# Lcrypto/mod-interleaveavx_multithreads-FAID

Hardware: AMD Instinct MI355X
Metric: decoded Gb/s @ 10 iters, 50G-PON LDPC; FER match vs AVX512 ref (higher is better)
Workload: dtype i8

## Files before the change

include/lnsfaid.h:

```cpp
#ifndef LNSFAID_H
#define LNSFAID_H

#include <stddef.h>
#include <stdint.h>

#ifdef __cplusplus
extern "C" {
#endif

#define LNSFAID_GROUP 32

#define LNSFAID_OK 0
#define LNSFAID_E_INVAL (-1)
#define LNSFAID_E_CODE (-2)
#define LNSFAID_E_NOMEM (-3)
#define LNSFAID_E_HIP (-4)
#define LNSFAID_E_NODEVICE (-5)
#define LNSFAID_E_INTERNAL (-6)

typedef struct lnsfaid_code {
    int32_t n_var;
    int32_t n_check;
    int32_t n_edges;
    int32_t z;
// ... 281 lines not shown
int lnsfaid_allreduce_counters(lnsfaid_ctx* ctx, uint64_t counters[4]);

int lnsfaid_select_kernel(lnsfaid_ctx* ctx, int32_t rows_per_lane);
int lnsfaid_kernel_rows_per_lane(const lnsfaid_ctx* ctx);

int lnsfaid_select_waves(lnsfaid_ctx* ctx, int32_t waves_per_codeword);
int lnsfaid_kernel_waves(const lnsfaid_ctx* ctx);

#define LNSFAID_MSG_REGISTERS 1
#define LNSFAID_MSG_HBM 2
int lnsfaid_select_message_store(lnsfaid_ctx* ctx, int32_t where);
int lnsfaid_message_store(const lnsfaid_ctx* ctx);

#define LNSFAID_ZERO_SHIFT_ON 1
#define LNSFAID_ZERO_SHIFT_OFF 2
#define LNSFAID_ZERO_SHIFT_LOOP 3
#define LNSFAID_ZERO_SHIFT_STATIC 4
#define LNSFAID_ZERO_SHIFT_WINDOWED 5
int lnsfaid_select_zero_shift(lnsfaid_ctx* ctx, int32_t mode);
int lnsfaid_zero_shift_groups(const lnsfaid_ctx* ctx, int32_t* groups, int32_t n);
int lnsfaid_window_free(const lnsfaid_ctx* ctx);
int lnsfaid_code_zero_shift_order(const lnsfaid_code* code, int32_t* groups, int32_t* order);

int lnsfaid_code_bf_walk(const lnsfaid_code* code, int32_t col_weight, uint32_t* full, uint32_t* flipped, uint32_t* fixed, int32_t* info);

int lnsfaid_kernel_residency(lnsfaid_ctx* ctx, int32_t* workgroups_per_cu, int32_t* lds_limit);


int lnsfaid_kernel_time(lnsfaid_ctx* ctx, double* out_ms, uint64_t* out_launches, int32_t reset);

void* lnsfaid_stream(lnsfaid_ctx* ctx);

const char* lnsfaid_strerror(int err);
const char* lnsfaid_last_hip_error(void);
const char* lnsfaid_version(void);

#ifdef __cplusplus
}
#endif
#endif
```

mod-interleaveavx_multithreads-faid_amd/csrc/lnsfaid_capi.hip:

```cpp
#include <hip/hip_runtime.h>

#include <dlfcn.h>
#include <rccl/rccl.h>

#include <cstdio>
#include <cstdlib>
#include <cstring>
#include <new>
#include <vector>

#include "lnsfaid_device.h"
#include "lnsfaid_line.h"
#include "lnsfaid_burst.h"
#include "lnsfaid_quantise.h"
#include "lnsfaid_swar.h"
#include "lnsfaid_launch.h"

#include <atomic>
#include <chrono>
#include <condition_variable>
#include <mutex>
#include <thread>
struct LfCombiner;
static thread_local char g_hip_err[256] = "";
// ... 45 lines not shown
    int32_t* d_status[2] = { nullptr, nullptr };
    uint32_t* d_remaining = nullptr;
    int32_t* d_live = nullptr;
    unsigned long long* d_counters = nullptr;
    uint32_t* h_remaining = nullptr;
    unsigned long long* h_counters = nullptr;
    int8_t* d_io_in = nullptr;
    int8_t* d_io_out = nullptr;
    lnsfaid_group_stats* d_io_stats = nullptr;
    lnsfaid_codeword_stats* d_io_cw_stats = nullptr;
    uint8_t* d_pk_in = nullptr;
    uint32_t* d_pk_out = nullptr;
    lnsfaid_group_stats* d_pk_stats = nullptr;
    uint32_t* d_ln_payload = nullptr;
    lnsfaid_line_stats* d_ln_stats = nullptr;
    LfBurstDesc* d_burst_desc = nullptr;
    LfBurstDesc* h_burst_desc = nullptr;
    uint32_t* d_burst_ones = nullptr;
    int early_stop = LNSFAID_STOP_GROUP;
    int rows_per_lane = 0;
    int waves_per_cw = 0;
    int msg_store = 0;
    int zero_shift = 0;
    mutable int static_code = -1;
    struct LfCombiner* comb = nullptr;
    int comb_slot = -1;
    const void* checked_fn[6] = {};
    int resident_wg[4] = {}, lds_wg[4] = {};
    void* comm = nullptr;
    bool comm_owned = false;
    unsigned long long* d_reduce = nullptr;
    double kernel_ms = 0.0;
    uint64_t kernel_launches = 0;
    uint32_t* d_fe_seeds = nullptr;
    unsigned long long* d_fe_draws = nullptr;
    int8_t* d_fe_codeword = nullptr;
    int8_t* d_fe_frames = nullptr;
    int8_t* d_fe_input = nullptr;
    size_t fe_frames_streams = 0;
    int fe_interleave = 1;
    int fe_exact = 0;
    int fe_prefec = 0;
    unsigned long long* d_fe_prefec_frames = nullptr;
    unsigned long long* d_fe_prefec_acc = nullptr;
    uint2* d_cap_cnt = nullptr;
    unsigned long long* d_cap_meta = nullptr;
// ... 321 lines not shown
    return LNSFAID_OK;
}

extern "C" int lnsfaid_create(lnsfaid_ctx** out, const lnsfaid_code* code, const lnsfaid_cfg* cfg, int32_t device,
                              size_t max_groups)
{
    if (!out || !code || !cfg || max_groups == 0 || max_groups > ((size_t)1 << 24)) return LNSFAID_E_INVAL;
    *out = nullptr;
    lnsfaid_ctx* ctx = new (std::nothrow) lnsfaid_ctx();
    if (!ctx) return LNSFAID_E_NOMEM;
    ctx->device = device;
    ctx->max_groups = max_groups;
    if (const char* e = getenv("LNSFAID_ROWS_PER_LANE"))
        ctx->rows_per_lane = (e[0] == '2') ? 2 : 0;
    if (const char* e = getenv("LNSFAID_WAVES_PER_CODEWORD"))
        ctx->waves_per_cw = (e[0] == '2') ? 2 : 0;
    if (const char* e = getenv("LNSFAID_FRONTEND_EXACT"))
        ctx->fe_exact = (e[0] == '1') ? 1 : 0;
    if (const char* e = getenv("LNSFAID_MSG_STORE"))
        ctx->msg_store = (e[0] == 'h') ? LNSFAID_MSG_HBM : ((e[0] == 'r') ? LNSFAID_MSG_REGISTERS : 0);
    if (const char* e = getenv("LNSFAID_ZERO_SHIFT"))
        ctx->zero_shift = (e[0] == 'o' && e[1] == 'f') ? LNSFAID_ZERO_SHIFT_OFF
                          : (e[0] == 'l' ? LNSFAID_ZERO_SHIFT_LOOP : (e[0] == 'w' ? LNSFAID_ZERO_SHIFT_WINDOWED : 0));
    g_live_contexts.fetch_add(1, std::memory_order_relaxed);
    const int rc = create_impl(ctx, code, cfg);
    if (rc) { lnsfaid_destroy(ctx); return rc; }
    ctx->comb_slot = comb_join(ctx);
    *out = ctx;
    return LNSFAID_OK;
}

extern "C" int lnsfaid_set_cfg(lnsfaid_ctx* ctx, const lnsfaid_cfg* cfg)
{
    if (!ctx || !cfg) return LNSFAID_E_INVAL;
    LfDevCfg n;
    int rc = build_cfg(cfg, &n);
    if (rc) return rc;
    rc = check_code_for_method(&ctx->hcode, n.method);
    if (rc) return rc;
    if (memcmp(&n, &ctx->hcfg, sizeof(n)) == 0) return LNSFAID_OK;
    HIP_TRY(hipSetDevice(ctx->device));
    HIP_TRY(hipStreamSynchronize(ctx->stream));
    if (n.W != ctx->hcfg.W) {
        build_wcols(&ctx->hcode, n.W);
        HIP_TRY(hipMemcpy(ctx->d_code, &ctx->hcode, sizeof(LfDevCode), hipMemcpyHostToDevice));
    }
// ... 66 lines not shown
static int layer_zero_groups(const lnsfaid_ctx* ctx, int br) { return (ctx->hcode.zinst[br] >> 8) & 0xff; }
static bool zero_shift_possible(const lnsfaid_ctx* ctx)
{
    if (!use_kernel4(ctx) || use_kernel5(ctx) || !use_msg_registers(ctx)) return false;
    if (ctx->hcfg.method < 1 || ctx->hcfg.method > 5) return false;
    for (int br = 0; br < ctx->hcode.nbr; ++br)
        if (layer_zero_groups(ctx, br) >= 1) return true;
    return false;
}
static bool use_zero_shift(const lnsfaid_ctx* ctx) { return ctx->zero_shift != LNSFAID_ZERO_SHIFT_OFF && zero_shift_possible(ctx); }

static bool static_layers_possible(const lnsfaid_ctx* ctx)
{
    if (ctx->static_code < 0) ctx->static_code = lf_decode4s_matches(&ctx->hcode);
    return ctx->static_code == 1 && zero_shift_possible(ctx);
}
static bool use_static_layers(const lnsfaid_ctx* ctx)
{
    return use_zero_shift(ctx) && ctx->zero_shift != LNSFAID_ZERO_SHIFT_LOOP && static_layers_possible(ctx);
}
static bool use_window_free(const lnsfaid_ctx* ctx)
{
    return use_static_layers(ctx) && ctx->zero_shift != LNSFAID_ZERO_SHIFT_WINDOWED && ctx->hcfg.floor_iter_thresh < 0;
}

extern "C" int lnsfaid_select_zero_shift(lnsfaid_ctx* ctx, int32_t mode)
{
    if (!ctx || mode < 0 || mode > LNSFAID_ZERO_SHIFT_WINDOWED) return LNSFAID_E_INVAL;
    if ((mode == LNSFAID_ZERO_SHIFT_ON || mode == LNSFAID_ZERO_SHIFT_LOOP) && !zero_shift_possible(ctx)) return LNSFAID_E_INVAL;
    if ((mode == LNSFAID_ZERO_SHIFT_STATIC || mode == LNSFAID_ZERO_SHIFT_WINDOWED) && !static_layers_possible(ctx)) return LNSFAID_E_INVAL;
    ctx->zero_shift = mode;
    return LNSFAID_OK;
}

extern "C" int lnsfaid_zero_shift_groups(const lnsfaid_ctx* ctx, int32_t* groups, int32_t n)
{
    if (!ctx || n < 0 || (n > 0 && !groups)) return LNSFAID_E_INVAL;
    const bool on = use_zero_shift(ctx);
    for (int br = 0; br < n; ++br) groups[br] = (on && br < ctx->hcode.nbr) ? layer_zero_groups(ctx, br) : 0;
    return on ? (use_static_layers(ctx) ? 2 : 1) : 0;
}

extern "C" int lnsfaid_window_free(const lnsfaid_ctx* ctx)
{
    if (!ctx) return LNSFAID_E_INVAL;
    return use_window_free(ctx) ? 1 : 0;
// ... 53 lines not shown
static bool cw_possible(const lnsfaid_ctx* ctx) { return ctx->waves_per_cw != 2 && use_kernel4(ctx); }

static bool packed_kernel(const lnsfaid_ctx* ctx) { return use_kernel4(ctx) && !use_kernel5(ctx); }

enum { LF_ENTRY_GROUP = LNSFAID_STOP_GROUP, LF_ENTRY_CW = LNSFAID_STOP_CODEWORD, LF_ENTRY_PACKED = 2 , LF_ENTRY_LINE = 4, LF_ENTRY_BURST };
static int decode_entry(int rule, bool packed) { return rule + (packed ? LF_ENTRY_PACKED : 0); }
struct LfInst {
    const void* fn;
    int threads;
};

static LfInst select_kernel(const lnsfaid_ctx* ctx, int entry)
{
    const int m = ctx->hcfg.method, ef = ctx->hcfg.ef, rm = use_msg_registers(ctx) ? 1 : 0;
    LfInst k = { nullptr, lf_decode4_threads() };
    switch (entry) {
    case LF_ENTRY_PACKED + LF_ENTRY_GROUP: k.fn = lf_decode4p_func(m, ef, rm, 0); break;
    case LF_ENTRY_PACKED + LF_ENTRY_CW: k.fn = lf_decode4p_func(m, ef, rm, 1); break;
    case LF_ENTRY_CW: if (cw_possible(ctx)) k.fn = lf_decode4cw_func(m, ef, rm); break;
    case LF_ENTRY_LINE: k.fn = lf_decode4l_func(m, ef, rm); break;
    case LF_ENTRY_BURST: k.fn = lf_decode4b_func(m, ef, rm); break;
    default:
        if (use_kernel5(ctx)) { k.fn = lf_decode5_func(m); k.threads = lf_decode5_threads(); }
        else if (use_window_free(ctx)) k.fn = lf_decode4w_func(m);
        else if (use_static_layers(ctx)) k.fn = lf_decode4s_func(m);
        else if (use_zero_shift(ctx)) k.fn = lf_decode4z_func(m);
        else if (use_kernel4(ctx)) k.fn = lf_decode4_func(m, ef, rm);
        else { k.fn = lf_decode_func(m, ctx->hcfg.uniform_w); k.threads = lf_decode_threads(); }
    }
    return k;
}

extern "C" int lnsfaid_select_message_store(lnsfaid_ctx* ctx, int32_t where)
{
    if (!ctx || where < 0 || where > LNSFAID_MSG_HBM) return LNSFAID_E_INVAL;
    if (where == LNSFAID_MSG_REGISTERS && !msg_registers_possible(ctx)) return LNSFAID_E_INVAL;
    ctx->msg_store = where;
    return LNSFAID_OK;
}

extern "C" int lnsfaid_message_store(const lnsfaid_ctx* ctx)
{
    if (!ctx) return LNSFAID_E_INVAL;
    if (!use_kernel4(ctx)) return LNSFAID_MSG_HBM;
    return use_msg_registers(ctx) ? LNSFAID_MSG_REGISTERS : LNSFAID_MSG_HBM;
}
// ... 431 lines not shown
            std::lock_guard<std::mutex> lk(cb->m);
            cb->slots[slot].state = LF_SLOT_FREE;
            cb->members -= 1;
            last = cb->members == 0;
            if (last) cb->stop = true;
            cb->cv_work.notify_all();
        }
        if (!last) return;
        if (g_comb[cb->device] == cb) g_comb[cb->device] = nullptr;
    }
    for (auto& th : cb->worker) if (th.joinable()) th.join();
    static const bool trace = getenv("LNSFAID_TRACE") != nullptr;
    if (trace && cb->batches)
        fprintf(stderr, "[lnsfaid] call combiner of device %d: %llu calls in %llu batches (%.1f per batch); per batch %.3f ms gathering, %.3f ms copies + decode\n",
                cb->device, (unsigned long long)cb->calls, (unsigned long long)cb->batches, (double)cb->calls / (double)cb->batches,
                cb->gather_ms / (double)cb->batches, cb->device_ms / (double)cb->batches);
    for (auto P : cb->pool) if (P) lnsfaid_destroy(P);
    if (cb->h_in) { (void)hipHostFree(cb->h_in); (void)hipHostFree(cb->h_out); (void)hipHostFree(cb->h_status); (void)hipHostFree(cb->h_stats); }
    delete cb;
}

static int comb_decode(lnsfaid_ctx* ctx, const int8_t* fixInput, int8_t* decodedBits, lnsfaid_group_stats* stats, int rule, int* rc_out)
{
    if (ctx->comb_slot < 0 || ctx->rows_per_lane != 0 || ctx->msg_store != 0 || ctx->waves_per_cw != 0 || ctx->zero_shift != 0) return 0;
    LfCombiner* cb = ctx->comb;
    const int slot = ctx->comb_slot;
    {
        std::lock_guard<std::mutex> lk(cb->m);
        if (cb->dead || cb->members < LF_COMB_MIN_MEMBERS || !cb->h_in) return 0;
        if (memcmp(&cb->code, &ctx->hcode, sizeof(LfDevCode)) != 0) return 0;
    }
    memcpy(cb->h_in + (size_t)slot * cb->group_bytes, fixInput, cb->group_bytes);
    int rc;
    {
        std::unique_lock<std::mutex> lk(cb->m);
        LfSlot& s = cb->slots[slot];
        s.cfg = ctx->hcfg;
        s.rule = rule;
        s.state = LF_SLOT_PENDING;
        cb->pending += 1;
        cb->cv_work.notify_all();
        if (!cb->cv_done.wait_for(lk, std::chrono::seconds(120), [&] { return s.state == LF_SLOT_DONE; })) {
            snprintf(g_hip_err, sizeof(g_hip_err), "call combiner: no result after 120 s");
            *rc_out = LNSFAID_E_INTERNAL;
            return 1;
        }
        rc = s.rc;
// ... 1624 lines not shown
```

mod-interleaveavx_multithreads-faid_amd/csrc/lnsfaid_launch.h:

```cpp
#ifndef LNSFAID_LAUNCH_H
#define LNSFAID_LAUNCH_H

#include <hip/hip_runtime.h>

#include <stdint.h>

#include "lnsfaid.h"

struct LfDevCode;
struct LfBurstDesc;

extern "C" {

const void* lf_decode_func(int method, int uniform_w);
int lf_decode_threads(void);
hipError_t lf_launch_count_errors(const int8_t* decoded, const int8_t* input_bits, int n_var, int k_info, size_t n_cw,
                                  unsigned long long* out, hipStream_t stream);
const void* lf_decode4_func(int method, int ef, int rm);
int lf_decode4_threads(void);
int lf_decode4_rm_layers(void);
const void* lf_decode4cw_func(int method, int ef, int rm);
const void* lf_decode4p_func(int method, int ef, int rm, int per_codeword);
hipError_t lf_launch_unpack_llr4(const uint8_t* d_llr4, int8_t* d_fix, size_t n_values, hipStream_t stream);
hipError_t lf_launch_pack_bits(const int8_t* d_decoded, uint32_t* d_bits, size_t n_values, hipStream_t stream);
hipError_t lf_launch_count_errors_packed(const uint32_t* d_bits, const uint32_t* d_msg, int n_var, int k_info, size_t n_cw,
                                         unsigned long long* out, hipStream_t stream);
const void* lf_decode4l_func(int method, int ef, int rm);
const void* lf_decode4b_func(int method, int ef, int rm);
int lf_decode4z_inst(int deg, int zg);
const void* lf_decode4z_func(int method);
int lf_decode4s_matches(const LfDevCode* code);
const void* lf_decode4s_func(int method);
const void* lf_decode4w_func(int method);
const void* lf_decode5_func(int method);
int lf_decode5_threads(void);

hipError_t lf_launch_frontend(const uint32_t* d_seeds, const unsigned long long* d_draws, int n_streams, int mod_type, float sigma_ch,
                              float scale, const int8_t* d_codeword, const int8_t* d_frames, int n_var, int n_check, int interleave,
                              int fast, int8_t* d_fix, int count_limit, unsigned long long* d_frame_cnt, hipStream_t stream);
hipError_t lf_frontend_fastpath_scan(double* d_out2, hipStream_t stream);
void lf_frontend_fastpath_assumed(double* eps2);
hipError_t lf_launch_prefec(const float* d_rx, const int8_t* d_sent, size_t n_groups, int mod_type, int n_var, int n_check,
                            int interleave, int scope, unsigned long long* d_out, hipStream_t stream);
hipError_t lf_launch_prefec_fold(unsigned long long* d_frame_cnt, size_t n_streams, unsigned long long* d_acc, hipStream_t stream);
hipError_t lf_launch_capture(const int8_t* d_fix, const int8_t* d_decoded, const int8_t* d_sent, size_t n_groups, int n_var, int n_check,
                             uint32_t skip, uint32_t cap, uint2* d_cnt, uint32_t* d_slots, lnsfaid_error_record* d_records,
                             int8_t* d_payload, unsigned long long* d_meta, unsigned long long* d_out, hipStream_t stream);
hipError_t lf_launch_fec_status(const LfDevCode* d_code, int n_var, int packed, const void* d_fix, const void* d_decided,
                                const int8_t* d_sent, size_t n_groups, lnsfaid_fec_record* d_records, int want_sent,
                                unsigned long long* d_acc, hipStream_t stream);
hipError_t lf_launch_demap(const float* d_rx, size_t n_groups, int mod_type, float scale, int n_var, int n_check, int interleave,
                           int packed, void* d_out, hipStream_t stream);
hipError_t lf_launch_encode(const LfDevCode* d_code, int n_check, const uint32_t* d_bsup, const uint32_t* d_bsup_off, const int8_t* d_in,
                            const unsigned long long* d_keys, size_t n_groups, int8_t* d_out, int8_t* d_info, hipStream_t stream);
hipError_t lf_launch_encode_line(const LfDevCode* d_code, int n_check, const uint32_t* d_bsup, const uint32_t* d_bsup_off,
                                 const uint32_t* d_payload, size_t n_codewords, uint32_t* d_line, uint32_t* d_bits, hipStream_t stream);
// ... 33 lines not shown
```

mod-interleaveavx_multithreads-faid_amd/csrc/lnsfaid_static50.h:

```cpp
#ifndef LNSFAID_STATIC50_H
#define LNSFAID_STATIC50_H

#include "lnsfaid_gpon_base.h"
#include "lnsfaid_swar.h"

#define SW50_LAYERS LNSFAID_GPON_BLOCK_ROWS

struct Sw50Layer {
    int deg, nz;
    uint32_t s4[SW_MAX_DEG];
    uint32_t cb256[SW_MAX_DEG];
};
struct Sw50Code {
    Sw50Layer layer[SW50_LAYERS];
};

constexpr Sw50Code sw50_build()
{
    struct Circ { int cb, shift; };
    constexpr int deg[SW50_LAYERS] = LNSFAID_GPON_ROW_DEG;
    constexpr Circ base[SW50_LAYERS][LNSFAID_GPON_MAX_DEG] = LNSFAID_GPON_BASE;
    Sw50Code c = {};
    for (int br = 0; br < SW50_LAYERS; ++br) {
        int n = 0;
// ... 15 lines not shown
template <int BR>
struct Sw50Tab {
    static_assert(BR >= 0 && BR < SW50_LAYERS, "layer of the 50G-PON code");
    static constexpr Sw50Layer L = sw50_build().layer[BR];
    static constexpr int DEG = L.deg, NZ = L.nz;
    uint32_t sbv;
    SW_MFN uint32_t s4(int j) const { return L.s4[j]; }
    SW_MFN uint32_t cb256(int j) const { return L.cb256[j]; }
    SW_MFN uint32_t sb_dyn4(uint32_t idx4) const
    {
#if SW_DEV
        return (uint32_t)__builtin_amdgcn_ds_bpermute((int)idx4, (int)sbv);
#else
        return (L.cb256[idx4 >> 2] << 16) | L.s4[idx4 >> 2];
#endif
    }
};
template <int BR>
struct SwTabStatic<Sw50Tab<BR>> {
    static constexpr bool value = true;
    static constexpr int nz = Sw50Tab<BR>::NZ;
};

constexpr int sw50_most_identities()
{
    constexpr Sw50Code c = sw50_build();
    int best = 0;
    for (int br = 1; br < SW50_LAYERS; ++br)
        if (c.layer[br].nz > c.layer[best].nz) best = br;
    return best;
}
#define SW50_CHECK_LAYER sw50_most_identities()

template <int BR>
SW_FN uint32_t sw50_row_parity(const SwLds& lds, uint32_t lane)
{
    typedef Sw50Tab<BR> Tab;
    constexpr int DEG = Tab::DEG, NZ = Tab::NZ;
    const Tab tab = Tab();
    const uint32_t tid4 = lane << 2;
    uint32_t ad[DEG], rq[DEG], ld[DEG];
#pragma unroll
    for (int j = 0; j < DEG; ++j) {
        const uint32_t x4 = tid4 + tab.s4(j);
        ad[j] = j < NZ ? tid4 : x4 & 0xfcu;
        rq[j] = j < NZ ? 0u : x4 >> 8;
// ... 31 lines not shown
```

mod-interleaveavx_multithreads-faid_amd/csrc/lnsfaid_swar.h:

```cpp
#ifndef LNSFAID_SWAR_H
#define LNSFAID_SWAR_H

#include <stdint.h>

#if defined(__HIPCC__)
#define SW_DEV 1
#define SW_FN __device__ __forceinline__
#define SW_HD __host__ __device__ __forceinline__
#else
#define SW_DEV 0
#define SW_FN static inline
#define SW_HD static inline
#endif

#define SW_MAX_DEG 24
#ifndef SW_ILP
#define SW_ILP 4
#endif

#if SW_DEV
#define SW_SCHED_FENCE() __builtin_amdgcn_sched_barrier(0)
#else
#define SW_SCHED_FENCE() ((void)0)
#endif
// ... 432 lines not shown
    const bool has1 = j0 + 1 < NJ, has2 = j0 + 2 < NJ, has3 = j0 + 3 < NJ;
    const uint32_t a = has1 ? sw_bitop3<SW_TT_SEL>(c55, m[0], m[1]) : m[0];
    const uint32_t b = has3 ? sw_bitop3<SW_TT_SEL>(c55, m[2], m[3]) : m[2];
    const uint32_t q = has2 ? sw_bitop3<SW_TT_SEL>(c33, a, b) : a;
    ns[j0 >> 3] = (j0 & 4) ? sw_bitop3<SW_TT_SEL>(c0f, ns[j0 >> 3], q) : q;
}

SW_FN uint32_t sw_plane_bit(const SwLds& lds, uint32_t era_plane, uint32_t a)
{
    const uint32_t v = (a & ~255u) | ((a >> 2) & 63u) | ((a & 3u) << 6);
    return (lds.rd32(era_plane + ((v >> 5) << 2)) >> (v & 31u)) & 1u;
}

#if SW_DEV
#define SW_MFN __device__ __forceinline__
#else
#define SW_MFN inline
#endif
struct SwNoXch {
    SW_MFN void put(int, uint32_t) const {}
    SW_MFN uint32_t get(int) const { return 0u; }
    SW_MFN void barrier() const {}
};
#define SW_OWN(j) (WAVES == 1 || (((j) & 1) == WAVE))

template <class Tab>
struct SwTabStatic {
    static constexpr bool value = false;
    static constexpr int nz = 0;
};

#define SW_PAIRS_PASS1 1
#define SW_PAIRS_PASS2 2
#define SW_PAIRS_ROW 4
#define SW_PAIRS_ALL (SW_PAIRS_PASS1 | SW_PAIRS_PASS2 | SW_PAIRS_ROW)
#define SW_FORM_NOWIN 1
#define SW_FORM_FRESH 2
#define SW_FORM_VK 4
#define SW_FORM_MUL 8
template <int METHOD, int DEG, bool ERA = false, int WAVES = 1, int WAVE = 0, int ZG = 0, int PAIRS = 0, int FORM = 0, class Tab, class Xch = SwNoXch>
SW_FN SwRow sw_layer_step(const SwLds& lds, const Tab& tab, const SwParams& p, const SwK& K, uint32_t lane, int deg, SwRow cur, bool fresh,
                          uint32_t rowpar, bool lme, uint32_t era_edges = 0u, uint32_t era_plane = 0u, const Xch& xch = Xch())
{
    constexpr bool NOWIN = (FORM & SW_FORM_NOWIN) != 0, FRESH = (FORM & SW_FORM_FRESH) != 0;
    constexpr bool VK = (FORM & SW_FORM_VK) != 0, MULF = (FORM & SW_FORM_MUL) != 0;
    static_assert(FORM == 0 || (WAVES == 1 && !ERA), "iteration forms: one-wave, non-erasing instances");
    static_assert(!NOWIN || METHOD != 0, "the normalised min-sum rows read no table after the search");
    static_assert(WAVES == 1 || !ERA, "the erasing variant is built for one wave per codeword only");
    static_assert(!ERA || METHOD == 2, "the erasure exists in Decode_FAID only");
    static_assert(ZG == 0 || (DEG > 0 && WAVES == 1 && !ERA && SW_ILP * ZG <= DEG), "rotation-free groups: per-degree, one-wave, non-erasing instances");
    constexpr bool STATIC = SwTabStatic<Tab>::value;
    static_assert(!STATIC || (ZG == 0 && DEG > 0 && WAVES == 1 && !ERA && SwTabStatic<Tab>::nz <= DEG), "static table view: per-degree, one-wave, non-erasing instances");
    constexpr int NZ = STATIC ? SwTabStatic<Tab>::nz : SW_ILP * ZG;
    constexpr int NJ = DEG > 0 ? DEG : SW_MAX_DEG;
    constexpr bool MINSUM = SW_MINSUM(METHOD);
    constexpr bool QUADS = WAVES == 1 && SW_ILP == 4 && DEG > 0;
    constexpr bool NSTREE = WAVES == 1 && SW_ILP == 4;
    constexpr bool EPAIRS = WAVES == 1 && DEG > 0 && SW_ILP % 2 == 0;
    constexpr bool EPAIRS1 = EPAIRS && (PAIRS & SW_PAIRS_PASS1), EPAIRS2 = EPAIRS && (PAIRS & SW_PAIRS_PASS2), RPAIRS = (PAIRS & SW_PAIRS_ROW) != 0;
    static_assert(!VK || DEG > 16, "the index decode of SW_FORM_VK: per-degree instances with edges in 16 .. 23");
    const uint32_t c78 = (VK && !MINSUM) ? 0x78787878u : K.c78;
    const uint32_t c01 = K.cbit[0], c80 = K.cbit[7], c7f = K.c7f, c0642 = K.c0642, cfc = K.cfc, sel_sign = K.sel_sign;
    const uint32_t tid4 = MULF ? lane : lane << 2;
#define SW_MASK7(x) (MULF ? sw_mask7_mul((x), sel_sign, K.c100) : sw_mask7((x), sel_sign))
#define SW_SHL8(x) (MULF ? sw_shl8_mul((x), K.c100) : (x) << 8)
    uint32_t s4j[NJ], cbj[NJ];
#pragma unroll
    for (int j = 0; j < NJ; ++j) { s4j[j] = (DEG > 0 || j < deg) ? tab.s4(j) : 0u; cbj[j] = (DEG > 0 || j < deg) ? tab.cb256(j) : 0u; }

    const uint32_t c2o = cur.cw & 0x07070707u, c1o = (cur.cw >> 3) & 0x07070707u;
    const uint32_t kp = 0x08080808u - c2o, kn = 0x08080808u + c2o;
    const uint32_t bias = MINSUM ? 0u : 0x06040200u;
    const uint32_t kt_lo = sw_perm(kn, kp, 0x05010400u) + (MINSUM ? 0u : 0x02020000u), kt_hi = sw_perm(kn, kp, 0x07030602u) + (MINSUM ? 0u : 0x06060404u);
    const uint32_t tt_lo = K.tt_lo, tt_hi = K.tt_hi;
    const uint32_t k_fresh = 0x08080808u + bias;

// ... 2 lines not shown
    if (!FRESH && !fresh && WAVE == 0) {
        const uint32_t a0 = cur.pa[0] & 0xffffu, a1 = cur.pa[0] >> 16, a2 = cur.pa[1] & 0xffffu, a3 = cur.pa[1] >> 16;
        SW_SCHED_FENCE();
        const uint32_t g0 = lds.rd8(a0), g1 = lds.rd8(a1), g2 = lds.rd8(a2), g3 = lds.rd8(a3);
        const uint32_t mneg = MULF ? sw_mask6_mul(cur.cw, sel_sign, K.c100) : sw_mask7(cur.cw << 1, sel_sign);
        padd = sw_bitop3<SW_TT_SEL>(mneg, c1o, c2o); psub = sw_bitop3<SW_TT_SEL>(mneg, c2o, c1o);
        SW_SCHED_FENCE();
        const uint32_t r = (MULF ? sw_gather4_perm(g0, g1, g2, g3) : sw_gather4(g0, g1, g2, g3)) + padd - psub;
        const uint32_t rh = sw_opaque(r >> 8);
        lds.wr8(a0, r); lds.wr8(a1, rh); lds.wr8(a2, r >> 16); lds.wr8(a3, rh >> 16);
    }
#endif
    if (WAVES == 2) xch.barrier();

    SW_SCHED_FENCE();
    uint32_t tb[NJ], ts[NJ], ms[NJ], ad[NJ], rq[NJ], ld[NJ];
    uint32_t t1 = 0xffffffffu, t2 = 0xffffffffu, ta[5] = { 0xffffffffu, 0xffffffffu, 0xffffffffu, 0xffffffffu, 0xffffffffu };
    uint32_t sx = 0;

#pragma unroll
    for (int j = 0; j < NJ; ++j) {
        if (j < NZ) {
            ad[j] = STATIC ? tid4 : tid4 | cbj[j];
        } else if ((DEG > 0 || j < deg) && SW_OWN(j)) {
            const uint32_t x4 = tid4 + s4j[j];
#if SW_DEV
            uint32_t a;
            if (STATIC) a = x4 & cfc;
            else asm("v_and_or_b32 %0, %1, %2, %3" : "=v"(a) : "v"(x4), "v"(cfc), "s"(cbj[j]));
#else
            const uint32_t a = STATIC ? x4 & cfc : (x4 & cfc) | cbj[j];
#endif
            ad[j] = a; rq[j] = x4 >> 8;
        }
    }
#define SW_COL(j) (STATIC ? cbj[j] : 0u)
#pragma unroll
    for (int j = 0; j < NJ; ++j)
        if ((DEG > 0 || j < deg) && SW_OWN(j)) ld[j] = lds.rd32(ad[j], SW_COL(j));
    SW_SCHED_FENCE();
#pragma unroll
    for (int j0 = 0; j0 < NJ; j0 += SW_ILP) {
        uint32_t r_[SW_ILP], x_[SW_ILP], s_[SW_ILP], k_[SW_ILP], a_[SW_ILP], i_[SW_ILP], u_[SW_ILP];
#define SW_EDGES(...) _Pragma("unroll") for (int g = 0; g < SW_ILP; ++g) { const int j = j0 + g; if (j < NJ && (DEG > 0 || j < deg) && SW_OWN(j)) { __VA_ARGS__ } }
#define SW_MASK_SHIFTS(EPAIRS, SRC, PRE)                                                                                                 \
        uint64_t sh_[SW_ILP / 2 + 1];                                                                                                    \
        if (EPAIRS) {                                                                                                                    \
            _Pragma("unroll") for (int g0 = 0; g0 < SW_ILP; g0 += 2) {                                                                   \
                _Pragma("unroll") for (int g = g0; g < g0 + 2; ++g) { const int j = j0 + g; if (j < NJ) { PRE } }                       \
                if (j0 + g0 + 1 < NJ) sh_[g0 >> 1] = sw_shl8x2(SRC(g0, j0 + g0), SRC(g0 + 1, j0 + g0 + 1));                              \
                else if (j0 + g0 < NJ) sh_[g0 >> 1] = SW_SHL8(SRC(g0, j0 + g0));                                                           \
            }                                                                                                                            \
        } else {                                                                                                                         \
            SW_EDGES(PRE)                                                                                                                \
        }
#define SW_MASK_EXPAND(EPAIRS, DST, SRC)                                                                                                 \
        if (EPAIRS) {                                                                                                                    \
            _Pragma("unroll") for (int g = 0; g < SW_ILP; ++g) {                                                                         \
                const int j = j0 + g;                                                                                                    \
                if (j < NJ) DST(g, j) = (g & 1) ? sw_mask7_hi(SRC(g, j), sh_[g >> 1], sel_sign) : sw_mask7_lo(SRC(g, j), sh_[g >> 1], sel_sign); \
            }                                                                                                                            \
        } else {                                                                                                                         \
            SW_EDGES(DST(g, j) = sw_mask7(SRC(g, j), sel_sign);)                                                                         \
        }
#define SW_P1_TS(g, j) ts[j]
#define SW_P1_MS(g, j) ms[j]
#define SW_P2_MO(g, j) mo[g]
        _Pragma("unroll") for (int g = SW_ILP - 1; g >= 0; --g) { const int j = j0 + g; if (j < NJ && (DEG > 0 || j < deg) && SW_OWN(j)) r_[g] = j < NZ ? ld[j] : sw_alignbyte(ld[j], ld[j], rq[j]); }
        if (FRESH) {
            SW_EDGES(x_[g] = 0u; s_[g] = c0642; k_[g] = k_fresh;)
        } else {
            SW_EDGES(x_[g] = (j & 7) ? cur.x[j >> 3] >> (j & 7) : cur.x[j >> 3];)
            SW_EDGES(s_[g] = sw_bitop3<SW_TT_ANDOR>(x_[g], c01, c0642);)
            SW_EDGES(k_[g] = sw_perm(kt_hi, kt_lo, s_[g]);)
        }
        if ((j0 + SW_ILP < NJ ? j0 + SW_ILP : NJ) <= NZ) { _Pragma("unroll") for (int g = SW_ILP - 1; g >= 0; --g) if (j0 + g < NJ) tb[j0 + g] = r_[g] + k_[g]; }
        else { SW_EDGES(tb[j] = r_[g] + k_[g];) }
        if (ERA) {
            SW_EDGES(x_[g] &= c01;)
            SW_EDGES(
                if ((era_edges >> j) & 1u) {
                    uint32_t em = 0, match = 0;
                    _Pragma("unroll") for (int k = 0; k < 4; ++k) {
                        const uint32_t a = ad[j] + ((rq[j] + (uint32_t)k) & 3u);
                        em |= sw_plane_bit(lds, era_plane, a) ? (0xffu << (8 * k)) : 0u;
                        const uint32_t pold = (k & 1) ? cur.pa[k >> 1] >> 16 : cur.pa[k >> 1] & 0xffffu;
                        match |= (!fresh && a == pold) ? (0xffu << (8 * k)) : 0u;
                    }
                    const uint32_t en_true = r_[g] - (padd & match) + (psub & match);
                    const uint32_t neg01 = ~((en_true + 0x08080808u) >> 7) & c01;
                    tb[j] = sw_bitop3<SW_TT_SEL>(em, c80 + bias, tb[j]);
// ... 115 lines not shown
#else
    for (int k = 0; k < 4; ++k) sbk[k] = WAVE == 0 ? tab.sb_dyn4((VK ? idx8 >> (8 * k + 1) : idx4 >> (8 * k)) & 0x7cu) : 0u;
#endif
    SW_SCHED_FENCE();

    const SwUpd2 u2 = sw_update2_consts<MINSUM>(c2n, fm, bias);
    const uint32_t cm27 = (WAVES == 2 || VK) ? 0u - 0x27272727u : K.cm27;
    uint32_t ns[3] = { 0u, 0u, 0u };
    uint32_t cbit[8];
#pragma unroll
    for (int e = 0; e < 8; ++e) cbit[e] = K.cbit[e];
#define SW_PASS2_ARITH(J0, EN)                                                                                       \
    {                                                                                                                \
        const int j0 = (J0);                                                                                         \
        uint32_t d_[SW_ILP], zb[SW_ILP], mo[SW_ILP], lm[SW_ILP];                                                     \
        SW_EDGES(d_[g] = sw_upd2_d(ms[j], u2);)                                                                      \
        SW_EDGES(zb[g] = sw_upd2_zb(tb[j], d_[g], u2);)                                                              \
        {                                                                                                            \
            SW_MASK_SHIFTS(EPAIRS2, SW_P2_MO, mo[g] = sw_upd2_out<MINSUM>(zb[g], d_[g], u2);)                        \
            SW_MASK_EXPAND(EPAIRS2, SW_P2_MO, SW_P2_MO)                                           \
        }                                                                                                            \
        SW_EDGES(lm[g] = sw_upd2_limit<MINSUM>(ms[j], d_[g], u2, c80);)                                              \
        SW_EDGES(EN[g] = sw_upd2_en(mo[g], lm[g], zb[g], d_[g], cm27);)                                              \
        SW_EDGES(if (j >= NZ) EN[g] = sw_alignbyte(EN[g], EN[g], 4u - rq[j]);)                                       \
        if (NSTREE) sw_sign_quad<NJ>(ns, ms, j0, deg, DEG > 0, K.c55, K.c33, K.c0f);                                 \
        else SW_EDGES(sw_sign_edge(ns, ms[j], j, cbit[j & 7]);)                                                      \
    }
#define SW_PASS2_STORE(J0, EN)                                                                                       \
    {                                                                                                                \
        const int j0 = (J0);                                                                                         \
        SW_EDGES(lds.wr32(ad[j], EN[g], SW_COL(j));)                                                                 \
    }
    uint32_t en0[SW_ILP], en1[SW_ILP];
    SW_PASS2_ARITH(0, en0)
    SW_SCHED_FENCE();
#pragma unroll
    for (int k = 0; k < 4; ++k)
        pa[k] = sw_node_addr(tid4 + sbk[k] + ((uint32_t)k << 8));
#ifdef SW_EXP_NO_ARGMIN
    gk0 = ld[0] & 0xffu; gk1 = ld[1] & 0xffu; gk2 = ld[2] & 0xffu; gk3 = ld[3] & 0xffu;
#else
    if (WAVE == 0) { gk0 = lds.rd8(pa[0]); gk1 = lds.rd8(pa[1]); gk2 = lds.rd8(pa[2]); gk3 = lds.rd8(pa[3]); }
#endif
    if (WAVES == 2 && WAVE == 0) {
        xch.put(0, c2n); xch.put(1, fm);
        xch.barrier();
    }
    SW_SCHED_FENCE();
    SW_PASS2_STORE(0, en0)
    if (SW_ILP < NJ) { SW_PASS2_ARITH(SW_ILP, en1) SW_PASS2_STORE(SW_ILP, en1) }
    SW_SCHED_FENCE();
    const uint32_t oh8 = sw_perm(K.oh_hi, K.oh_lo, idx & 0x07070707u);
    uint32_t nm3, nm4;
    if (RPAIRS && (DEG == 0 || DEG > 16)) {
// ... 88 lines not shown
```

mod-interleaveavx_multithreads-faid_amd/pyabi.py:

```python
import ctypes as C
import os

HERE = os.path.dirname(os.path.abspath(__file__))
LIB_PATH = os.path.join(HERE, "csrc", "liblnsfaid.so")

GROUP = 32
MSG_REGISTERS, MSG_HBM = 1, 2
ZERO_SHIFT_ON, ZERO_SHIFT_OFF, ZERO_SHIFT_LOOP, ZERO_SHIFT_STATIC, ZERO_SHIFT_WINDOWED = 1, 2, 3, 4, 5
STOP_GROUP, STOP_CODEWORD = 0, 1
SHORTEN_TAIL, SHORTEN_HEAD = 0, 1
LINE_HARD, LINE_LLR4 = 0, 1
LINE_CAPTURE_UNCORRECTABLE, LINE_CAPTURE_WRONG = 1, 2


class Code(C.Structure):
    _fields_ = [
        ("n_var", C.c_int32),
        ("n_check", C.c_int32),
        ("n_edges", C.c_int32),
        ("z", C.c_int32),
        ("puncture_tail", C.c_int32),
        ("nb_degres", C.c_int32),
        ("deg", C.POINTER(C.c_int32)),
        ("deg_rows", C.POINTER(C.c_int32)),
# ... 151 lines not shown
    "lnsfaid_encode_device": (C.c_int, [C.c_void_p, C.c_void_p, C.c_size_t, C.c_void_p]),
    "lnsfaid_encode": (C.c_int, [C.c_void_p, C.c_void_p, C.c_size_t, C.c_void_p]),
    "lnsfaid_frontend_random_frames": (C.c_int, [C.c_void_p, C.POINTER(C.c_uint64), C.c_size_t]),
    "lnsfaid_io_buffers": (C.c_int, [C.c_void_p, C.POINTER(C.c_void_p), C.POINTER(C.c_void_p), C.POINTER(C.c_void_p)]),
    "lnsfaid_read_stats": (C.c_int, [C.c_void_p, C.c_void_p, C.c_size_t]),
    "lnsfaid_host_register": (C.c_int, [C.c_void_p, C.c_size_t]),
    "lnsfaid_host_unregister": (C.c_int, [C.c_void_p]),
    "lnsfaid_comm_unique_id": (C.c_int, [C.c_void_p]),
    "lnsfaid_comm_init": (C.c_int, [C.c_void_p, C.c_int32, C.c_int32, C.c_void_p]),
    "lnsfaid_comm_attach": (C.c_int, [C.c_void_p, C.c_void_p]),
    "lnsfaid_comm_destroy": (C.c_int, [C.c_void_p]),
    "lnsfaid_allreduce_counters": (C.c_int, [C.c_void_p, C.POINTER(C.c_uint64)]),
    "lnsfaid_select_kernel": (C.c_int, [C.c_void_p, C.c_int32]),
    "lnsfaid_kernel_rows_per_lane": (C.c_int, [C.c_void_p]),
    "lnsfaid_select_waves": (C.c_int, [C.c_void_p, C.c_int32]),
    "lnsfaid_frontend_set_exact": (C.c_int, [C.c_void_p, C.c_int32]),
    "lnsfaid_frontend_fastpath_bounds": (C.c_int, [C.c_void_p, C.POINTER(C.c_double), C.POINTER(C.c_double)]),
    "lnsfaid_kernel_waves": (C.c_int, [C.c_void_p]),
    "lnsfaid_select_message_store": (C.c_int, [C.c_void_p, C.c_int32]),
    "lnsfaid_message_store": (C.c_int, [C.c_void_p]),
    "lnsfaid_select_zero_shift": (C.c_int, [C.c_void_p, C.c_int32]),
    "lnsfaid_zero_shift_groups": (C.c_int, [C.c_void_p, C.POINTER(C.c_int32), C.c_int32]),
    "lnsfaid_window_free": (C.c_int, [C.c_void_p]),
    "lnsfaid_code_zero_shift_order": (C.c_int, [C.POINTER(Code), C.POINTER(C.c_int32), C.POINTER(C.c_int32)]),
    "lnsfaid_code_bf_walk": (C.c_int, [C.POINTER(Code), C.c_int32, C.POINTER(C.c_uint32), C.POINTER(C.c_uint32), C.POINTER(C.c_uint32),
                                      C.POINTER(C.c_int32)]),
    "lnsfaid_kernel_residency": (C.c_int, [C.c_void_p, C.POINTER(C.c_int32), C.POINTER(C.c_int32)]),
    "lnsfaid_kernel_time": (C.c_int, [C.c_void_p, C.POINTER(C.c_double), C.POINTER(C.c_uint64), C.c_int32]),
    "lnsfaid_stream": (C.c_void_p, [C.c_void_p]),
    "lnsfaid_strerror": (C.c_char_p, [C.c_int]),
    "lnsfaid_last_hip_error": (C.c_char_p, []),
    "lnsfaid_version": (C.c_char_p, []),
}


def bind(lib, symbols):
    for name, (res, args) in symbols.items():
        fn = getattr(lib, name)
        fn.restype = res
        fn.argtypes = args
    return lib


_lib = None


# ... 962 lines not shown

    def message_store(self):
        return self.lib.lnsfaid_message_store(self.ctx)

    def select_zero_shift(self, mode):
        self._check(self.lib.lnsfaid_select_zero_shift(self.ctx, mode), "lnsfaid_select_zero_shift")

    def zero_shift_groups(self, n_layers=32):
        zg = (C.c_int32 * n_layers)()
        on = self.lib.lnsfaid_zero_shift_groups(self.ctx, zg, n_layers)
        self._check(min(on, 0), "lnsfaid_zero_shift_groups")
        return on >= 1, list(zg)

    def static_layers(self):
        on = self.lib.lnsfaid_zero_shift_groups(self.ctx, None, 0)
        self._check(min(on, 0), "lnsfaid_zero_shift_groups")
        return on == 2

    def window_free(self):
        on = self.lib.lnsfaid_window_free(self.ctx)
        self._check(min(on, 0), "lnsfaid_window_free")
        return on == 1

    def kernel_residency(self):
        wg, lim = C.c_int32(), C.c_int32()
        self._check(self.lib.lnsfaid_kernel_residency(self.ctx, C.byref(wg), C.byref(lim)), "lnsfaid_kernel_residency")
        return wg.value, lim.value

    def kernel_time(self, reset=False):
        ms = C.c_double()
        n = C.c_uint64()
        self._check(self.lib.lnsfaid_kernel_time(self.ctx, C.byref(ms), C.byref(n), 1 if reset else 0), "lnsfaid_kernel_time")
        return ms.value, n.value

    def close(self):
        if self.ctx:
            self.lib.lnsfaid_destroy(self.ctx)
            self.ctx = C.c_void_p()

    def __del__(self):
        try:
            self.close()
        except Exception:
            pass
```

Before: 89.90.

## Precompute per-lane edge address/rotation words and prefetch them per layer

Adds a new decode kernel variant (4e) that reads precomputed per-lane LDS address and byte-rotation words for every rotating edge from a constant device image. The words for the next layer are prefetched into registers during the current layer's write pass. This replaces the per-edge add/shift/mask address and rotation arithmetic inside the layer step. It costs extra VGPRs for the word buffers and global/constant loads, which could lower occupancy. The variant is on by default when the window-free static path applies, and the combiner path stays available.

Result: faster. 90.83, median of 6 (+1.0%).

```diff
diff --git a/include/lnsfaid.h b/include/lnsfaid.h
--- a/include/lnsfaid.h
+++ b/include/lnsfaid.h
@@ -327,6 +327,9 @@
 int lnsfaid_window_free(const lnsfaid_ctx* ctx);
 int lnsfaid_code_zero_shift_order(const lnsfaid_code* code, int32_t* groups, int32_t* order);
 
+int lnsfaid_select_edge_words(lnsfaid_ctx* ctx, int32_t on);
+int lnsfaid_edge_words(const lnsfaid_ctx* ctx);
+
 int lnsfaid_code_bf_walk(const lnsfaid_code* code, int32_t col_weight, uint32_t* full, uint32_t* flipped, uint32_t* fixed, int32_t* info);
 
 int lnsfaid_kernel_residency(lnsfaid_ctx* ctx, int32_t* workgroups_per_cu, int32_t* lds_limit);
diff --git a/mod-interleaveavx_multithreads-faid_amd/csrc/lnsfaid_capi.hip b/mod-interleaveavx_multithreads-faid_amd/csrc/lnsfaid_capi.hip
--- a/mod-interleaveavx_multithreads-faid_amd/csrc/lnsfaid_capi.hip
+++ b/mod-interleaveavx_multithreads-faid_amd/csrc/lnsfaid_capi.hip
@@ -91,6 +91,7 @@
     int waves_per_cw = 0;
     int msg_store = 0;
     int zero_shift = 0;
+    int edge_words = 1;
     mutable int static_code = -1;
     struct LfCombiner* comb = nullptr;
     int comb_slot = -1;
@@ -458,6 +459,8 @@
     if (const char* e = getenv("LNSFAID_ZERO_SHIFT"))
         ctx->zero_shift = (e[0] == 'o' && e[1] == 'f') ? LNSFAID_ZERO_SHIFT_OFF
                           : (e[0] == 'l' ? LNSFAID_ZERO_SHIFT_LOOP : (e[0] == 'w' ? LNSFAID_ZERO_SHIFT_WINDOWED : 0));
+    if (const char* e = getenv("LNSFAID_EDGE_WORDS"))
+        ctx->edge_words = (e[0] == 'o' && e[1] == 'f') ? 0 : 1;
     g_live_contexts.fetch_add(1, std::memory_order_relaxed);
     const int rc = create_impl(ctx, code, cfg);
     if (rc) { lnsfaid_destroy(ctx); return rc; }
@@ -570,6 +573,21 @@
 static bool use_window_free(const lnsfaid_ctx* ctx)
 {
     return use_static_layers(ctx) && ctx->zero_shift != LNSFAID_ZERO_SHIFT_WINDOWED && ctx->hcfg.floor_iter_thresh < 0;
+}
+
+static bool use_edge_words(const lnsfaid_ctx* ctx) { return ctx->edge_words != 0 && use_window_free(ctx); }
+
+extern "C" int lnsfaid_select_edge_words(lnsfaid_ctx* ctx, int32_t on)
+{
+    if (!ctx || on < 0 || on > 1) return LNSFAID_E_INVAL;
+    ctx->edge_words = on;
+    return LNSFAID_OK;
+}
+
+extern "C" int lnsfaid_edge_words(const lnsfaid_ctx* ctx)
+{
+    if (!ctx) return LNSFAID_E_INVAL;
+    return use_edge_words(ctx) ? 1 : 0;
 }
 
 extern "C" int lnsfaid_select_zero_shift(lnsfaid_ctx* ctx, int32_t mode)
@@ -669,6 +687,7 @@
     case LF_ENTRY_BURST: k.fn = lf_decode4b_func(m, ef, rm); break;
     default:
         if (use_kernel5(ctx)) { k.fn = lf_decode5_func(m); k.threads = lf_decode5_threads(); }
+        else if (use_edge_words(ctx)) k.fn = lf_decode4e_func(m);
         else if (use_window_free(ctx)) k.fn = lf_decode4w_func(m);
         else if (use_static_layers(ctx)) k.fn = lf_decode4s_func(m);
         else if (use_zero_shift(ctx)) k.fn = lf_decode4z_func(m);
@@ -1146,7 +1165,7 @@
 
 static int comb_decode(lnsfaid_ctx* ctx, const int8_t* fixInput, int8_t* decodedBits, lnsfaid_group_stats* stats, int rule, int* rc_out)
 {
-    if (ctx->comb_slot < 0 || ctx->rows_per_lane != 0 || ctx->msg_store != 0 || ctx->waves_per_cw != 0 || ctx->zero_shift != 0) return 0;
+    if (ctx->comb_slot < 0 || ctx->rows_per_lane != 0 || ctx->msg_store != 0 || ctx->waves_per_cw != 0 || ctx->zero_shift != 0 || ctx->edge_words != 1) return 0;
     LfCombiner* cb = ctx->comb;
     const int slot = ctx->comb_slot;
     {
diff --git a/mod-interleaveavx_multithreads-faid_amd/csrc/lnsfaid_kernel4e.hip b/mod-interleaveavx_multithreads-faid_amd/csrc/lnsfaid_kernel4e.hip
--- /dev/null
+++ b/mod-interleaveavx_multithreads-faid_amd/csrc/lnsfaid_kernel4e.hip
@@ -0,0 +1,161 @@
+#include <hip/hip_runtime.h>
+
+#define LF4_MAIN_STEP main_step4e
+#define LF4_DIRTY_CHECK(c, lane) dirty4e(lane)
+#include "lnsfaid_frame4.h"
+#include "lnsfaid_static50.h"
+#include "lnsfaid_launch.h"
+
+static_assert(SW50_LAYERS == LF4_RM_LAYERS, "one register of every message vector per layer");
+
+__device__ const Sw50EdgeImage lf4e_edge_words = sw50_edge_image();
+
+__device__ __forceinline__ bool dirty4e(int lane)
+{
+    const SwLds lds = SwLds();
+    asm volatile("; lf4e check stage 1");
+    const uint32_t w1 = sw50_row_parity<SW50_CHECK_LAYER>(lds, (uint32_t)lane);
+    if (__ballot((w1 & 0x80808080u) != 0u) != 0ull) return true;
+    asm volatile("; lf4e check stage 2");
+    const uint32_t w0 = sw50_row_parity<0>(lds, (uint32_t)lane);
+    return __ballot((w0 & 0x80808080u) != 0u) != 0ull;
+}
+
+#define LF4E_EW(METHOD) ((METHOD) == 3 ? 0 : SW_FORM_EDGEW)
+#define LF4E_MIDDLE(METHOD) (SW_FORM_NOWIN | SW_FORM_VK | SW_FORM_MUL | LF4E_EW(METHOD))
+#define LF4E_FIRST(METHOD) (LF4E_MIDDLE(METHOD) | SW_FORM_FRESH)
+
+#define LF4E_MAX_GROUPS 6
+constexpr int LF4E_GROUPS0 = sw50_edge_groups(0);
+
+template <int BR>
+__device__ __forceinline__ void load_words4e(uint32_t lane16, int g, uint32_t* w)
+{
+    constexpr int G0 = sw50_edge_group_base(BR);
+    const uint4 v = *(const uint4*)((const char*)lf4e_edge_words.w + (size_t)((G0 + g) * SW50_EDGE_GROUP_WORDS * 4) + lane16);
+    w[4 * g] = v.x; w[4 * g + 1] = v.y; w[4 * g + 2] = v.z; w[4 * g + 3] = v.w;
+}
+
+template <int BR>
+struct Lf4eEw {
+    static constexpr int NZ = Sw50Tab<BR>::NZ;
+    static constexpr int NEXT = BR + 1 < SW50_LAYERS ? BR + 1 : 0;
+    static constexpr int NG = BR + 1 < SW50_LAYERS ? sw50_edge_groups(NEXT) : 0;
+    static constexpr int LAST = (Sw50Tab<BR>::DEG - 1) / SW_ILP * SW_ILP;
+    const uint32_t* cur;
+    uint32_t* next;
+    uint32_t lane16;
+    static constexpr int first_of(int j)
+    {
+        for (int i = NZ; i < j; ++i)
+            if (Sw50Tab<BR>::L.s4[i] == Sw50Tab<BR>::L.s4[j]) return i;
+        return j;
+    }
+    __device__ __forceinline__ uint32_t w(int j) const { return cur[j - NZ]; }
+    __device__ __forceinline__ uint32_t wa(int j) const { return cur[first_of(j) - NZ]; }
+    __device__ __forceinline__ void at(int point) const
+    {
+        const int g0 = point / SW_ILP, g1 = point == LAST ? NG : (g0 + 1 < NG ? g0 + 1 : NG);
+        __builtin_amdgcn_sched_barrier(0);
+#pragma unroll
+        for (int g = g0; g < g1; ++g) load_words4e<NEXT>(lane16, g, next);
+        __builtin_amdgcn_sched_barrier(0);
+    }
+};
+
+template <int METHOD, int FORM, int BR>
+__device__ __forceinline__ void layer4e(const uint32_t (*zsb)[32], SwRegs& R, const SwLds& lds, const SwParams& p, const SwK& K, int lane, uint32_t lane16,
+                                        bool fresh, uint32_t& tabv, uint32_t* w)
+{
+    typedef Sw50Tab<BR> Tab;
+    asm volatile("; lf4e layer %2" : "+v"(lane), "+v"(lane16) : "n"(BR));
+    uint32_t tabn = 0u;
+    if (BR + 1 < SW50_LAYERS) tabn = *(const uint32_t*)((const char*)zsb[BR + 1] + (lane & 0x7c));
+    Tab tab;
+    tab.sbv = tabv;
+    uint32_t wn[4 * LF4E_MAX_GROUPS];
+    const Lf4eEw<BR> ew = { w, wn, lane16 };
+    const SwRow zero = { { 0u, 0u, 0u }, 0u, { 0u, 0u } };
+    SwRow cur = (FORM & SW_FORM_FRESH) ? zero : regs_get(R, BR);
+    if (!(FORM & SW_FORM_FRESH)) asm volatile("" : "+v"(cur.cw));
+    SwRow st = sw_layer_step<METHOD, Tab::DEG, false, 1, 0, 0, SW_PAIRS_ALL, FORM>(lds, tab, p, K, (uint32_t)lane, Tab::DEG, cur,
+                                                                                  (FORM & SW_FORM_FRESH) ? true : fresh, 0u, false, 0u, 0u, SwNoXch(), ew);
+    asm volatile("" : "+v"(st.x[0]), "+v"(st.x[1]), "+v"(st.x[2]), "+v"(st.cw), "+v"(st.pa[0]), "+v"(st.pa[1]));
+    __builtin_amdgcn_sched_barrier(0);
+    regs_put(R, BR, st);
+    __builtin_amdgcn_sched_barrier(0);
+    tabv = tabn;
+#pragma unroll
+    for (int i = 0; i < 4 * Lf4eEw<BR>::NG; ++i) w[i] = wn[i];
+}
+
+template <int METHOD, int FORM>
+__device__ __forceinline__ void layers4e(const uint32_t (*zsb)[32], SwRegs& R, const SwLds& lds, const SwParams& p, const SwK& K, int lane, uint32_t lane16,
+                                         bool fresh, uint32_t tabv, uint32_t* w)
+{
+#define LF4E_LAYER(BR) layer4e<METHOD, FORM, BR>(zsb, R, lds, p, K, lane, lane16, fresh, tabv, w);
+    LF4E_LAYER(0) LF4E_LAYER(1) LF4E_LAYER(2) LF4E_LAYER(3) LF4E_LAYER(4) LF4E_LAYER(5)
+    LF4E_LAYER(6) LF4E_LAYER(7) LF4E_LAYER(8) LF4E_LAYER(9) LF4E_LAYER(10) LF4E_LAYER(11)
+#undef LF4E_LAYER
+}
+
+template <int METHOD, bool ERA, bool RM>
+__device__ __forceinline__ void main_step4e(CCode c, CCfg f, const LfDevCode* gc, SwRow* __restrict__ rows, SwRegs& R, int lane, int it, const uint32_t* sP,
+                                            bool have_par, bool lme, uint32_t era_plane)
+{
+    static_assert(RM && !ERA, "built for the messages-in-registers, non-erasing instances only");
+    (void)c; (void)rows; (void)era_plane; (void)sP; (void)have_par; (void)lme;
+    it = __builtin_amdgcn_readfirstlane(it);
+    const uint32_t lane16 = (uint32_t)lane << 4;
+    uint32_t w[4 * LF4E_MAX_GROUPS];
+#pragma unroll
+    for (int g = 0; g < (LF4E_EW(METHOD) ? LF4E_GROUPS0 : 0); ++g) load_words4e<0>(lane16, g, w);
+    SwK K = sw_consts((uint32_t)it);
+    const bool first = (it == 1);
+    const int itx = (it >= 1 && it <= 5) ? it - 1 : 5;
+    SwParams p;
+    p.lut_lo = f->lut_lo[itx][0]; p.lut_hi = f->lut_hi[itx][0];
+    p.ef_lo = f->lut_ef_lo[itx][0]; p.ef_hi = f->lut_ef_hi[itx][0];
+    p.f1 = f->factor_1; p.f2 = f->factor_2;
+    p.window = false;
+    p.ef_tables = f->ef >= 1;
+    if (LF4_OMS(METHOD)) sw_oms_tables(p);
+    {
+        uint32_t tm[4];
+        sw_therm2msg_tables(LF4_OMS(METHOD) ? p.oms_lo[0] : p.lut_lo, LF4_OMS(METHOD) ? p.oms_hi[0] : p.lut_hi, tm);
+#pragma unroll
+        for (int k = 0; k < 4; ++k) K.tm[k] = sw_vconst(tm[k], (uint32_t)it);
+    }
+    K.c100 = sw_vconst(0x100u, (uint32_t)it);
+    const int lane_arg = lane << 2;
+    const SwLds lds = SwLds();
+    uint32_t z = 0u;
+    asm volatile("" : "+s"(z));
+    const uint32_t (*zsb)[32] = (const uint32_t (*)[32])((const char*)gc->zsbplain + z);
+    const uint32_t tabv = zsb[0][lane & 31];
+    __builtin_amdgcn_sched_barrier(0);
+    if (first) {
+        asm volatile("; lf4e first begin");
+        layers4e<METHOD, LF4E_FIRST(METHOD)>(zsb, R, lds, p, K, lane_arg, lane16, true, tabv, w);
+        asm volatile("; lf4e first end");
+    } else {
+        asm volatile("; lf4e middle begin");
+        layers4e<METHOD, LF4E_MIDDLE(METHOD)>(zsb, R, lds, p, K, lane_arg, lane16, false, tabv, w);
+        asm volatile("; lf4e middle end");
+    }
+}
+
+#define LF4_RULE GROUP
+
+template <int METHOD>
+__global__ __launch_bounds__(LF_T4, 2) void lnsfaid_decode4e_kernel(LfKernelArgs a_)
+{
+    constexpr bool RM = true, EF2 = false;
+    LF4_SPLIT_ARGS()
+    LF4_GROUP_FRAME(LF4_STAGE_INPUT, write_decoded, int8_t, N)
+}
+
+extern "C" const void* lf_decode4e_func(int method)
+{
+    LF4_METHOD_TABLE(lnsfaid_decode4e_kernel)
+}
diff --git a/mod-interleaveavx_multithreads-faid_amd/csrc/lnsfaid_launch.h b/mod-interleaveavx_multithreads-faid_amd/csrc/lnsfaid_launch.h
--- a/mod-interleaveavx_multithreads-faid_amd/csrc/lnsfaid_launch.h
+++ b/mod-interleaveavx_multithreads-faid_amd/csrc/lnsfaid_launch.h
@@ -32,6 +32,7 @@
 int lf_decode4s_matches(const LfDevCode* code);
 const void* lf_decode4s_func(int method);
 const void* lf_decode4w_func(int method);
+const void* lf_decode4e_func(int method);
 const void* lf_decode5_func(int method);
 int lf_decode5_threads(void);
 
diff --git a/mod-interleaveavx_multithreads-faid_amd/csrc/lnsfaid_static50.h b/mod-interleaveavx_multithreads-faid_amd/csrc/lnsfaid_static50.h
--- a/mod-interleaveavx_multithreads-faid_amd/csrc/lnsfaid_static50.h
+++ b/mod-interleaveavx_multithreads-faid_amd/csrc/lnsfaid_static50.h
@@ -61,6 +61,40 @@
     static constexpr int nz = Sw50Tab<BR>::NZ;
 };
 
+constexpr uint32_t sw50_edge_word_of(uint32_t s4, int lane)
+{
+    const uint32_t x = (uint32_t)lane + (s4 >> 2), rq = (x >> 6) & 3u;
+    return ((x & 63u) << 2) | rq | (((4u - rq) & 3u) << 8);
+}
+constexpr uint32_t sw50_edge_word(int layer, int edge, int lane) { return sw50_edge_word_of(sw50_build().layer[layer].s4[edge], lane); }
+constexpr int sw50_edge_groups(int layer) { return (sw50_build().layer[layer].deg - sw50_build().layer[layer].nz + 3) / 4; }
+constexpr int sw50_edge_group_base(int layer)
+{
+    int n = 0;
+    for (int br = 0; br < layer; ++br) n += sw50_edge_groups(br);
+    return n;
+}
+#define SW50_EDGE_GROUPS sw50_edge_group_base(SW50_LAYERS)
+#define SW50_EDGE_GROUP_WORDS 256
+struct Sw50EdgeImage {
+    uint32_t w[SW50_EDGE_GROUPS * SW50_EDGE_GROUP_WORDS];
+};
+constexpr Sw50EdgeImage sw50_edge_image()
+{
+    constexpr Sw50Code c = sw50_build();
+    Sw50EdgeImage im = {};
+    int g0 = 0;
+    for (int br = 0; br < SW50_LAYERS; ++br) {
+        const int rot = c.layer[br].deg - c.layer[br].nz;
+        for (int e = 0; e < rot; ++e)
+            for (int lane = 0; lane < 64; ++lane)
+                im.w[((g0 + e / 4) * 64 + lane) * 4 + e % 4] = sw50_edge_word_of(c.layer[br].s4[c.layer[br].nz + e], lane);
+        g0 += (rot + 3) / 4;
+    }
+    return im;
+}
+static_assert(SW50_EDGE_GROUPS == 56, "206 rotating edges in groups of four, layer by layer");
+
 constexpr int sw50_most_identities()
 {
     constexpr Sw50Code c = sw50_build();
diff --git a/mod-interleaveavx_multithreads-faid_amd/csrc/lnsfaid_swar.h b/mod-interleaveavx_multithreads-faid_amd/csrc/lnsfaid_swar.h
--- a/mod-interleaveavx_multithreads-faid_amd/csrc/lnsfaid_swar.h
+++ b/mod-interleaveavx_multithreads-faid_amd/csrc/lnsfaid_swar.h
@@ -478,6 +478,11 @@
     SW_MFN uint32_t get(int) const { return 0u; }
     SW_MFN void barrier() const {}
 };
+struct SwNoEw {
+    SW_MFN uint32_t w(int) const { return 0u; }
+    SW_MFN uint32_t wa(int) const { return 0u; }
+    SW_MFN void at(int) const {}
+};
 #define SW_OWN(j) (WAVES == 1 || (((j) & 1) == WAVE))
 
 template <class Tab>
@@ -494,9 +499,10 @@
 #define SW_FORM_FRESH 2
 #define SW_FORM_VK 4
 #define SW_FORM_MUL 8
-template <int METHOD, int DEG, bool ERA = false, int WAVES = 1, int WAVE = 0, int ZG = 0, int PAIRS = 0, int FORM = 0, class Tab, class Xch = SwNoXch>
+#define SW_FORM_EDGEW 16
+template <int METHOD, int DEG, bool ERA = false, int WAVES = 1, int WAVE = 0, int ZG = 0, int PAIRS = 0, int FORM = 0, class Tab, class Xch = SwNoXch, class Ew = SwNoEw>
 SW_FN SwRow sw_layer_step(const SwLds& lds, const Tab& tab, const SwParams& p, const SwK& K, uint32_t lane, int deg, SwRow cur, bool fresh,
-                          uint32_t rowpar, bool lme, uint32_t era_edges = 0u, uint32_t era_plane = 0u, const Xch& xch = Xch())
+                          uint32_t rowpar, bool lme, uint32_t era_edges = 0u, uint32_t era_plane = 0u, const Xch& xch = Xch(), const Ew& ew = Ew())
 {
     constexpr bool NOWIN = (FORM & SW_FORM_NOWIN) != 0, FRESH = (FORM & SW_FORM_FRESH) != 0;
     constexpr bool VK = (FORM & SW_FORM_VK) != 0, MULF = (FORM & SW_FORM_MUL) != 0;
@@ -508,6 +514,8 @@
     constexpr bool STATIC = SwTabStatic<Tab>::value;
     static_assert(!STATIC || (ZG == 0 && DEG > 0 && WAVES == 1 && !ERA && SwTabStatic<Tab>::nz <= DEG), "static table view: per-degree, one-wave, non-erasing instances");
     constexpr int NZ = STATIC ? SwTabStatic<Tab>::nz : SW_ILP * ZG;
+    constexpr bool EDGEW = (FORM & SW_FORM_EDGEW) != 0;
+    static_assert(!EDGEW || (STATIC && WAVES == 1 && !ERA), "edge words: static table views, one-wave, non-erasing instances");
     constexpr int NJ = DEG > 0 ? DEG : SW_MAX_DEG;
     constexpr bool MINSUM = SW_MINSUM(METHOD);
     constexpr bool QUADS = WAVES == 1 && SW_ILP == 4 && DEG > 0;
@@ -556,6 +564,9 @@
     for (int j = 0; j < NJ; ++j) {
         if (j < NZ) {
             ad[j] = STATIC ? tid4 : tid4 | cbj[j];
+        } else if (EDGEW) {
+            rq[j] = ew.wa(j);
+            ad[j] = rq[j] & cfc;
         } else if ((DEG > 0 || j < deg) && SW_OWN(j)) {
             const uint32_t x4 = tid4 + s4j[j];
 #if SW_DEV
@@ -600,7 +611,7 @@
 #define SW_P1_TS(g, j) ts[j]
 #define SW_P1_MS(g, j) ms[j]
 #define SW_P2_MO(g, j) mo[g]
-        _Pragma("unroll") for (int g = SW_ILP - 1; g >= 0; --g) { const int j = j0 + g; if (j < NJ && (DEG > 0 || j < deg) && SW_OWN(j)) r_[g] = j < NZ ? ld[j] : sw_alignbyte(ld[j], ld[j], rq[j]); }
+        _Pragma("unroll") for (int g = SW_ILP - 1; g >= 0; --g) { const int j = j0 + g; if (j < NJ && (DEG > 0 || j < deg) && SW_OWN(j)) r_[g] = j < NZ ? ld[j] : sw_alignbyte(ld[j], ld[j], EDGEW ? ew.w(j) : rq[j]); }
         if (FRESH) {
             SW_EDGES(x_[g] = 0u; s_[g] = c0642; k_[g] = k_fresh;)
         } else {
@@ -762,7 +773,7 @@
         }                                                                                                            \
         SW_EDGES(lm[g] = sw_upd2_limit<MINSUM>(ms[j], d_[g], u2, c80);)                                              \
         SW_EDGES(EN[g] = sw_upd2_en(mo[g], lm[g], zb[g], d_[g], cm27);)                                              \
-        SW_EDGES(if (j >= NZ) EN[g] = sw_alignbyte(EN[g], EN[g], 4u - rq[j]);)                                       \
+        SW_EDGES(if (j >= NZ) EN[g] = sw_alignbyte(EN[g], EN[g], EDGEW ? rq[j] >> 8 : 4u - rq[j]);)                  \
         if (NSTREE) sw_sign_quad<NJ>(ns, ms, j0, deg, DEG > 0, K.c55, K.c33, K.c0f);                                 \
         else SW_EDGES(sw_sign_edge(ns, ms[j], j, cbit[j & 7]);)                                                      \
     }
@@ -770,6 +781,7 @@
     {                                                                                                                \
         const int j0 = (J0);                                                                                         \
         SW_EDGES(lds.wr32(ad[j], EN[g], SW_COL(j));)                                                                 \
+        if (EDGEW) ew.at(j0);                                                                                        \
     }
     uint32_t en0[SW_ILP], en1[SW_ILP];
     SW_PASS2_ARITH(0, en0)
diff --git a/mod-interleaveavx_multithreads-faid_amd/pyabi.py b/mod-interleaveavx_multithreads-faid_amd/pyabi.py
--- a/mod-interleaveavx_multithreads-faid_amd/pyabi.py
+++ b/mod-interleaveavx_multithreads-faid_amd/pyabi.py
@@ -197,6 +197,8 @@
     "lnsfaid_select_zero_shift": (C.c_int, [C.c_void_p, C.c_int32]),
     "lnsfaid_zero_shift_groups": (C.c_int, [C.c_void_p, C.POINTER(C.c_int32), C.c_int32]),
     "lnsfaid_window_free": (C.c_int, [C.c_void_p]),
+    "lnsfaid_select_edge_words": (C.c_int, [C.c_void_p, C.c_int32]),
+    "lnsfaid_edge_words": (C.c_int, [C.c_void_p]),
     "lnsfaid_code_zero_shift_order": (C.c_int, [C.POINTER(Code), C.POINTER(C.c_int32), C.POINTER(C.c_int32)]),
     "lnsfaid_code_bf_walk": (C.c_int, [C.POINTER(Code), C.c_int32, C.POINTER(C.c_uint32), C.POINTER(C.c_uint32), C.POINTER(C.c_uint32),
                                       C.POINTER(C.c_int32)]),
@@ -1205,6 +1207,14 @@
         self._check(min(on, 0), "lnsfaid_window_free")
         return on == 1
 
+    def select_edge_words(self, on):
+        self._check(self.lib.lnsfaid_select_edge_words(self.ctx, 1 if on else 0), "lnsfaid_select_edge_words")
+
+    def edge_words(self):
+        on = self.lib.lnsfaid_edge_words(self.ctx)
+        self._check(min(on, 0), "lnsfaid_edge_words")
+        return on == 1
+
     def kernel_residency(self):
         wg, lim = C.c_int32(), C.c_int32()
         self._check(self.lib.lnsfaid_kernel_residency(self.ctx, C.byref(wg), C.byref(lim)), "lnsfaid_kernel_residency")
```
